# prj-beatrice/beatrice-vst

Hardware: AMD Instinct MI355X
Metric: audio frames/sec (24 kHz out, 10 ms hop) (higher is better)
Workload: dtype f32

## Files before the change

### beatrice-vst_amd/csrc/batch_tick.hip.h

```cpp
#pragma once

#ifdef BEATRICE_HIP_MEASUREMENT_BUILD
static unsigned long long g_tick_only_types = ~0ull;
#endif
template <int H>
bool tick_build_table_h(BeatriceBatch* b, const bool sparse) {
  using namespace tick;
  using O = Ops<H>;
  using Tab = typename O::Tab;
  using OpF2 = typename O::OpF2; using OpF3 = typename O::OpF3; using OpF4 = typename O::OpF4; using OpF5 = typename O::OpF5; using OpRB = typename O::OpRB;
  using OpOUT = typename O::OpOUT; using OpP1 = typename O::OpP1; using OpP23 = typename O::OpP23; using OpPOUT = typename O::OpPOUT; using OpINP = typename O::OpINP;
  using OpUP1 = typename O::OpUP1; using OpRES1A = typename O::OpRES1A; using OpRES1B = typename O::OpRES1B; using OpUP2 = typename O::OpUP2;
  using OpF4s = typename O::OpF4s; using OpF5s = typename O::OpF5s; using OpRBs = typename O::OpRBs; using OpP1s = typename O::OpP1s; using OpUP1s = typename O::OpUP1s;
  using T1 = typename O::T1; using T2 = typename O::T2; using T3 = typename O::T3; using T1s = typename O::T1s; using T2s = typename O::T2s;
  using GruQ = typename O::GruQ; using GruP = typename O::GruP; using GruQ1 = typename O::GruQ1; using GruP1 = typename O::GruP1;
  using GruQm = typename O::GruQm; using GruPm = typename O::GruPm;
  State& k = b->tk;
  if (sparse && !sparse_table_at(H)) { k.table_sparse_total = 0; return true; }
  auto tb = std::make_unique<typename O::Builder>();
  const PhoneWeights& pw = b->phone_m->w;
  const PitchWeights& qw = b->pitch_m->w;
  const WaveWeights& ww = b->wave_m->w;
  const PhoneState& ps = b->phone;
  const PitchState& qs = b->pitch;
  const WaveState& ws = b->wave;
  const int B = b->B;
  const Plan pl = k.plan;
#ifdef BEATRICE_HIP_MEASUREMENT_BUILD
  static const int drop = bhip::meas_env("BEATRICE_HIP_TICK_DROP") ? std::atoi(bhip::meas_env("BEATRICE_HIP_TICK_DROP")) : 0;
#else
  constexpr int drop = 0;
#endif
  auto keep = [](int group) { return ((drop >> group) & 1) == 0; };
#ifdef BEATRICE_HIP_MEASUREMENT_BUILD
  tb->only = g_tick_only_types;
#endif
  auto hp = [&](int) -> const int* { return nullptr; };
  auto conv = [&](const Ring& in, const Ring& out, const float* w, const float* bias, int stage) { return conv_args(in, out, w, bias, hp(stage), B); };
  static const int gru_passes_env = bhip::meas_env("BEATRICE_HIP_GRU_PASSES") ? std::atoi(bhip::meas_env("BEATRICE_HIP_GRU_PASSES")) : 0;
  const int gru_passes = gru_passes_env > 0 ? gru_passes_env : (B >= 512 ? 2 : 1);
  auto link_p = [&](int t) { return k.d_link_p + (size_t)t * B * 256; };
  auto link_q = [&](int t) { return k.d_link_q + (size_t)t * B * 128; };
  auto add_pgru = [&](int t) {
    if constexpr (H > 1) {
      GruArgs g{ps.rb[3], ps.h, pw.gru_wih, pw.gru_whh, pw.gru_bih, pw.gru_bhh, hp(Plan::PGRU), B, t, t + 1 < H ? link_p(t) : nullptr, t > 0 ? link_p(t - 1) : nullptr, k.h_link_dead, gru_passes};
      if (t == 0) tb->template add<T_PGRU>(GruP::info("phone.gru", g), g, GruP::grid(g), Plan::PGRU, keep(1), 19);
      else if (t == H - 1) tb->template add<T_PGRU1>(GruP1::info("phone.gru", g), g, GruP1::grid(g), Plan::PGRU, keep(1), 19);
      else if constexpr (H > 2) tb->template add<T_PGRUM>(GruPm::info("phone.gru", g), g, GruPm::grid(g), Plan::PGRU, keep(1), 19);
    }
  };
  auto add_qgru = [&](int t) {
    if constexpr (H > 1) {
      GruArgs g{qs.p[2], qs.h, qw.gru_wih, qw.gru_whh, qw.gru_bih, qw.gru_bhh, hp(Plan::QGRU), B, t, t + 1 < H ? link_q(t) : nullptr, t > 0 ? link_q(t - 1) : nullptr, k.h_link_dead, gru_passes};
      if (t == 0) tb->template add<T_QGRU>(GruQ::info("pitch.gru", g), g, GruQ::grid(g), Plan::QGRU, keep(1), 12);
      else if (t == H - 1) tb->template add<T_QGRU1>(GruQ1::info("pitch.gru", g), g, GruQ1::grid(g), Plan::QGRU, keep(1), 12);
      else if constexpr (H > 2) tb->template add<T_QGRUM>(GruQm::info("pitch.gru", g), g, GruQm::grid(g), Plan::QGRU, keep(1), 12);
    }
  };
  auto gru_at = [&](int point) {
    if constexpr (H == 2) { if (point == 2) add_pgru(1); if (point == 3) add_qgru(1); }
    if constexpr (H == 4) {
      if (point == 0) { add_pgru(1); add_qgru(1); }
      if (point == 1) { add_pgru(2); add_qgru(2); }
      if (point == 2) add_pgru(3);
      if (point == 3) add_qgru(3);
    }
  };
  add_pgru(0); add_qgru(0);
  if (!sparse) {
    { const ConvArgs a = conv(ps.f[3], ps.f[4], pw.f_w[3], pw.f_b[3], Plan::F5); tb->template add<T_F5>(OpF5::info("phone.f5", a), a, OpF5::grid(a), Plan::F5, keep(6), 30); }
    { const ConvArgs a = conv(qs.spec, qs.p[0], qw.p_w[0], qw.p_b[0], Plan::P1); tb->template add<T_P1>(OpP1::info("pitch.p1", a), a, OpP1::grid(a), Plan::P1, keep(2), 41); }
    { const ConvArgs a = conv(ps.f[2], ps.f[3], pw.f_w[2], pw.f_b[2], Plan::F4); tb->template add<T_F4>(OpF4::info("phone.f4", a), a, OpF4::grid(a), Plan::F4, keep(6), 28); }
    for (int i = 0; i < 4; ++i) {
      const ConvArgs a = conv(i == 0 ? ps.f[4] : ps.rb[i - 1], ps.rb[i], pw.rb_w[i], pw.rb_b[i], Plan::RB0 + i);
      tb->template add<T_RB>(OpRB::info("phone.rb", a), a, OpRB::grid(a), Plan::RB0 + i, keep(6), 39);
    }
  } else {
    { const ConvArgs a = conv(ps.f[3], ps.f[4], pw.f_w[3], pw.f_b[3], Plan::F5); tb->template add<T_F5S>(OpF5s::info("phone.f5", a), a, OpF5s::grid(a), Plan::F5, keep(6), 30); }
    { const ConvArgs a = conv(qs.spec, qs.p[0], qw.p_w[0], qw.p_b[0], Plan::P1); tb->template add<T_P1S>(OpP1s::info("pitch.p1", a), a, OpP1s::grid(a), Plan::P1, keep(2), 41); }
    { const ConvArgs a = conv(ps.f[2], ps.f[3], pw.f_w[2], pw.f_b[2], Plan::F4); tb->template add<T_F4S>(OpF4s::info("phone.f4", a), a, OpF4s::grid(a), Plan::F4, keep(6), 28); }
    for (int i = 0; i < 4; ++i) {
      const ConvArgs a = conv(i == 0 ? ps.f[4] : ps.rb[i - 1], ps.rb[i], pw.rb_w[i], pw.rb_b[i], Plan::RB0 + i);
      tb->template add<T_RBS>(OpRBs::info("phone.rb", a), a, OpRBs::grid(a), Plan::RB0 + i, keep(6), 39);
    }
  }
  for (int blk = 0; blk < B_NBLOCKS; ++blk) {
    const WaveState::Scratch& sc = ws.scr[blk];
    const int s0 = pl.blk(blk);
    const rc::BlockBArgs ba{sc.xa, ws.x[blk + 1], ww.q_w[blk], ww.q_b[blk], ww.o_w[blk], ww.o_b[blk], ws.d_kt[blk], ws.d_v[blk],
                            b->dev_view<int>(b->off.perm[blk]), b->dev_view<int>(b->off.tile_slot[blk]), hp(s0 + 1)};
    tb->template add<T_BLKB>(LaunchInfo{"wave.blk.b", 2.0 * B * H * (256.0 * 256 * 2 + 256.0 * 384 * 2), 4.0 * (2.0 * 256 * 256 + 2.0 * 256 * 384 + B * H * 3.0 * 256)}, ba,
                    dim3(ws.n_tiles_max, 1), s0 + 1, keep(5), 43.0);
    if (quads_on(b)) {
      const rc::BlockBqArgs bq{sc.xa, ws.x[blk + 1], ww.q_w[blk], ww.q_b[blk], ww.o_w[blk], ww.o_b[blk], ws.d_ktp[blk], ws.d_vp[blk],
                               b->dev_view<int>(b->off.qperm[blk]), b->dev_view<int>(b->off.qslot[blk]), hp(s0 + 1)};
      tb->template add<T_BLKBQ>(LaunchInfo{"wave.blk.bq", 0.0, 0.0}, bq, dim3(std::min(2 * ws.n_tiles_max, ws.n_slots), 1), s0 + 1, keep(5), 42.0);
    }
  }
  for (int blk = 0; blk < B_NBLOCKS; ++blk) {
    const rc::BlockAArgs aa{ws.x[blk], ws.scr[blk].xa, ww.c1_w[blk], ww.c1_b[blk], ww.c2_w[blk], ww.c2_b[blk], hp(pl.blk(blk)), B};
    switch (blk) {
      case 0: tb->template add<T_BLKA1>(rc::BlockAOp<1, H>::info(aa), aa, rc::BlockAOp<1, H>::grid(aa), pl.blk(blk), keep(5), 38); break;
      case 1: tb->template add<T_BLKA2>(rc::BlockAOp<2, H>::info(aa), aa, rc::BlockAOp<2, H>::grid(aa), pl.blk(blk), keep(5), 38); break;
      case 2: tb->template add<T_BLKA4>(rc::BlockAOp<4, H>::info(aa), aa, rc::BlockAOp<4, H>::grid(aa), pl.blk(blk), keep(5), 38); break;
      default: tb->template add<T_BLKA8>(rc::BlockAOp<8, H>::info(aa), aa, rc::BlockAOp<8, H>::grid(aa), pl.blk(blk), keep(5), 38); break;
    }
  }
  gru_at(0);
  { const VqArgs a{H, ps.raw, phone_vector_ring(ps), hp(Plan::VQ), ps.d_cbT, ps.d_cnorm, ps.d_vqk}; tb->template add<T_VQ>(LaunchInfo{"phone.vq", 0, 4.0 * B * H * 256}, a, dim3(B, 1), Plan::VQ, !ps.skip_vq, 9.0 * H, true); }
  {
    tst::StageArgs t1{}, t2{}, t3{};
    t1.in = ws.ya2; t1.out = ws.ya3; t2.in = ws.ya3; t2.out = ws.ya4; t3.in = ws.ya4;
    for (tst::StageArgs* t : {&t1, &t2, &t3}) { t->state = ws.tail.base; t->hop = nullptr; t->B = B; }
    t1.w[0] = ww.ra_w[1]; t1.b[0] = ww.ra_b[1]; t1.w[1] = ww.rb_w[1]; t1.b[1] = ww.rb_b[1]; t1.w[2] = ww.up_w[2]; t1.b[2] = ww.up_b[2];
    t2.w[0] = ww.ra_w[2]; t2.b[0] = ww.ra_b[2]; t2.w[1] = ww.rb_w[2]; t2.b[1] = ww.rb_b[2]; t2.w[2] = ww.up_w[3]; t2.b[2] = ww.up_b[3];
    t3.w[0] = ww.ra_w[3]; t3.b[0] = ww.ra_b[3]; t3.w[1] = ww.rb_w[3]; t3.b[1] = ww.rb_b[3];
    t3.fin_w = ww.fin_w; t3.fin_b = ww.fin_b; t3.d_out = ws.d_out; t3.io_stride = ws.io_stride;
    if (!sparse) {
      tb->template add<T_TAIL1>(T1::info(t1), t1, T1::grid(t1), pl.tail(), keep(4), 28, true);
      tb->template add<T_TAIL2>(T2::info(t2), t2, T2::grid(t2), pl.tail() + 1, keep(4), 11.5 * H, true);
    } else {
      tb->template add<T_TAIL1S>(T1s::info(t1), t1, T1s::grid(t1), pl.tail(), keep(4), 28, true);
      tb->template add<T_TAIL2S>(T2s::info(t2), t2, T2s::grid(t2), pl.tail() + 1, keep(4), 11.5 * H, true);
    }
    tb->template add<T_TAIL3>(T3::info(t3), t3, T3::grid(t3), pl.tail() + 2, keep(4), 6.5 * H, true);
  }
  gru_at(1);
  { PitchHeadArgs a = head_args(qw, qs); a.hop = hp(Plan::HEAD); tb->template add<T_HEAD>(head_info(qs), a, dim3((B + 7) / 8, 1), Plan::HEAD, keep(0), 7.5 * H); }
  { const ConvArgs a = conv(ps.f[1], ps.f[2], pw.f_w[1], pw.f_b[1], Plan::F3); tb->template add<T_F3>(OpF3::info("phone.f3", a), a, OpF3::grid(a), Plan::F3, keep(6), 15); }
  if (!sparse) { const ConvArgs a = conv(ws.x[4], ws.ya1, ww.up_w[0], ww.up_b[0], pl.up1()); tb->template add<T_UP1>(OpUP1::info("wave.up1", a), a, OpUP1::grid(a), pl.up1(), keep(7), 14); }
  else { const ConvArgs a = conv(ws.x[4], ws.ya1, ww.up_w[0], ww.up_b[0], pl.up1()); tb->template add<T_UP1S>(OpUP1s::info("wave.up1", a), a, OpUP1s::grid(a), pl.up1(), keep(7), 14); }
  { const ConvArgs a = conv(ws.yb1, ws.yc1, ww.rb_w[0], ww.rb_b[0], pl.up1() + 2); tb->template add<T_RES1B>(OpRES1B::info("wave.res1b", a), a, OpRES1B::grid(a), pl.up1() + 2, keep(7), 13); }
  { const ConvArgs a = conv(ws.ya1, ws.yb1, ww.ra_w[0], ww.ra_b[0], pl.up1() + 1); tb->template add<T_RES1A>(OpRES1A::info("wave.res1a", a), a, OpRES1A::grid(a), pl.up1() + 1, keep(7), 13); }
  { const ConvArgs a = conv(ws.yc1, ws.ya2, ww.up_w[1], ww.up_b[1], pl.up1() + 3); tb->template add<T_UP2>(OpUP2::info("wave.up2", a), a, OpUP2::grid(a), pl.up1() + 3, keep(7), 13); }
  { const ConvArgs a = conv(ps.f[0], ps.f[1], pw.f_w[0], pw.f_b[0], Plan::F2); tb->template add<T_F2>(OpF2::info("phone.f2", a), a, OpF2::grid(a), Plan::F2, keep(6), 15); }
  if constexpr (H == 1) { const GruArgs g{ps.rb[3], ps.h, pw.gru_wih, pw.gru_whh, pw.gru_bih, pw.gru_bhh, hp(Plan::PGRU), B, 0, nullptr, nullptr, nullptr, gru_passes}; tb->template add<T_PGRU>(GruP::info("phone.gru", g), g, GruP::grid(g), Plan::PGRU, keep(1), 19); }
  gru_at(2);
  { const ConvArgs a = conv(qs.h, qs.logits, qw.out_w, qw.out_b, Plan::POUT); tb->template add<T_POUT>(OpPOUT::info("pitch.out", a), a, OpPOUT::grid(a), Plan::POUT, keep(2), 11); }
  for (int i = 0; i < 2; ++i) {
    const ConvArgs a = conv(qs.p[i], qs.p[i + 1], qw.p_w[i + 1], qw.p_b[i + 1], Plan::P2 + i);
    tb->template add<T_P23>(OpP23::info("pitch.p23", a), a, OpP23::grid(a), Plan::P2 + i, keep(2), 10);
  }
  { const Ring phone_in{ws.d_phone, B_PHONE_CH, H, ws.front_slots}; ConvArgs a = conv(phone_in, ws.x[0], ww.inp_w, ww.inp_b, Plan::INP); a.res = ws.e; tb->template add<T_INP>(OpINP::info("wave.inp", a), a, OpINP::grid(a), Plan::INP, keep(3), 7.5); }
  if constexpr (H == 1) { const GruArgs g{qs.p[2], qs.h, qw.gru_wih, qw.gru_whh, qw.gru_bih, qw.gru_bhh, hp(Plan::QGRU), B, 0, nullptr, nullptr, nullptr, gru_passes}; tb->template add<T_QGRU>(GruQ::info("pitch.gru", g), g, GruQ::grid(g), Plan::QGRU, keep(1), 12); }
  gru_at(3);
  { FftArgs a = fft_args(qw, qs); a.hop = hp(Plan::FFT); tb->template add<T_FFT>(fft_info(qs), FftArgs2{a, B}, dim3((B + 1) / 2, H), Plan::FFT, keep(0), 8.7); }
  { const ConvArgs a = conv(ps.h, phone_out_ring(ps), pw.out_w, pw.out_b, Plan::OUT); tb->template add<T_OUT>(OpOUT::info("phone.out", a), a, OpOUT::grid(a), Plan::OUT, keep(3), 4.5); }
  { F1Args a = f1_args(pw, ps); a.hop = hp(Plan::F1); a.hop_publish = nullptr; a.hop_publish_wave = nullptr; tb->template add<T_F1>(f1_info(ps), F1Args2{a, B}, dim3((B + 1) / 2, H), Plan::F1, keep(0), 3.7); }
  { CondArgs a = cond_args(ww, ws); a.hop = hp(Plan::COND); a.hop_next_out = nullptr; tb->template add<T_COND>(cond_info(ws), a, dim3((B * H + 1) / 2, 1), Plan::COND, keep(0), 1.5); }
  if (!tb->ok) return false;
  static const int halves_mode = bhip::meas_env("BEATRICE_HIP_TICK_HALVES") ? std::atoi(bhip::meas_env("BEATRICE_HIP_TICK_HALVES")) : 2;
  {
    std::vector<fuse::WgDesc> desc;
    bool pinned[fuse::kMaxSpans];
    int group[fuse::kMaxSpans];
    for (int i = 0; i < tb->t.n_spans; ++i) {
      group[i] = -1;
      switch (tb->t.span[i].type) {
        case T_PGRU: case T_PGRU1: case T_PGRUM: pinned[i] = true; group[i] = 0; break;
        case T_QGRU: case T_QGRU1: case T_QGRUM: pinned[i] = true; group[i] = 1; break;
        case T_F2: case T_F3: case T_F4: case T_F5: case T_P1: case T_RB: case T_F4S: case T_F5S: case T_P1S: case T_RBS:
        case T_BLKA1: case T_BLKA2: case T_BLKA4: case T_BLKA8: case T_BLKB: case T_BLKBQ:
        case T_UP1: case T_UP1S: case T_RES1A: case T_RES1B: case T_UP2: case T_POUT: case T_P23: case T_INP: case T_OUT: pinned[i] = true; break;
        default: pinned[i] = false; break;
      }
    }
    if (halves_mode != 0 && !sparse) {
      desc = tb->two_halves(pinned, group, halves_mode == 4 ? 4 : 2);
    } else {
      desc = tb->in_span_order();
    }
    auto upload = [&](const std::vector<fuse::WgDesc>& v, DevBuf<fuse::WgDesc>& d_desc) {
      if (v.size() > d_desc.size() && !d_desc.alloc(v.size(), "tick dispatch order", false)) return false;
      if (!v.empty()) BHIP_TRY(hipMemcpy(d_desc, v.data(), sizeof(fuse::WgDesc) * v.size(), hipMemcpyHostToDevice));
      return true;
    };
    if (!sparse) {
      const std::vector<fuse::WgDesc> plain = tb->in_span_order();
      if (!upload(plain, k.d_desc_plain)) return false;
      k.table_total_plain = (int)plain.size();
      for (auto& row : k.range_n) for (int& n : row) n = 0;
      const int n_stages = pl.count();
      static const int range_halves_from = bhip::meas_env("BEATRICE_HIP_TICK_RANGE_HALVES") ? std::atoi(bhip::meas_env("BEATRICE_HIP_TICK_RANGE_HALVES")) : kRangeHalvesFrom;
      if (plain.size() <= 16384 && n_stages <= kMaxStages) {
        std::vector<fuse::WgDesc> all;
        for (int shape = 0; shape < 2; ++shape)
          for (int s0 = 0; s0 < n_stages; ++s0) {
            k.range_off[shape][s0] = all.size();
            const int occupied = shape == 0 ? s0 + 1 : n_stages - s0;
            if (halves_mode != 0 && occupied >= range_halves_from) {
              const std::vector<fuse::WgDesc> part = shape == 0 ? tb->two_halves(pinned, group, 2, 0, s0) : tb->two_halves(pinned, group, 2, s0, 255);
              all.insert(all.end(), part.begin(), part.end());
            } else {
              for (const fuse::WgDesc& d : plain) {
                const int stage = (d.arg >> 16) & 0xff;
                if (shape == 0 ? stage <= s0 : stage >= s0) all.push_back(d);
              }
            }
            k.range_n[shape][s0] = (int)(all.size() - k.range_off[shape][s0]);
          }
        if (!upload(all, k.d_desc_ranges)) return false;
      }
    }
    tb->t.total = (int)desc.size();
    if (!upload(desc, sparse ? k.d_desc_sparse : k.d_desc)) return false;
  }
  if (bhip::meas_env("BEATRICE_HIP_TICK_TRACE")) {
    if (!k.d_trace.alloc((size_t)3 * tb->t.total, "tick trace", false)) return false;
    tb->t.trace = k.d_trace;
// ... 530 lines not shown
```

### beatrice-vst_amd/csrc/rowchain.hip.h

```cpp
#pragma once
#include "meas_env.h"
#include <hip/hip_runtime.h>

#include <cstdlib>

#include "conv_gemm.hip.h"
#include "kernels_misc.hip.h"
#include "ring.h"
#include "spec_math.hip.h"

#ifdef RC_TIMING
__device__ unsigned long long* g_rc_stamps;
#define RC_STAMP(i) do { if (threadIdx.x == 0) g_rc_stamps[(size_t)blockIdx.x * 16 + (i)] = __builtin_readcyclecounter(); } while (0)
#else
#define RC_STAMP(i) do { } while (0)
#endif

namespace rc {

constexpr int NTHR = 512, NWAVE = 8;
constexpr int AS = B_HID + 8;
constexpr int TILE = 16 * AS;
constexpr int SS = B_KV_LEN + 8;
constexpr int STILE = 16 * SS;
__host__ __device__ constexpr int kpos(int k) { return (k & ~15) | ((k & 3) << 2) | ((k >> 2) & 3); }
constexpr int KSTEP = 4;
template <int ROWGROUPS >
__device__ __forceinline__ void piece_of(const int W, const int ln, int* r, int* q) {
  *r = 4 * (W % ROWGROUPS) + (ln >> 4); *q = 16 * (W / ROWGROUPS) + (ln & 15);
}
__device__ __forceinline__ int lane_koff(const int lane) { return 4 * (lane >> 4); }
__device__ __forceinline__ float4 lds_kblock(const float* __restrict__ p, const int kb) { return *reinterpret_cast<const float4*>(p + kb * 16); }
__device__ __forceinline__ void store_perm4(float* __restrict__ row, const int n0, const float v0, const float v1, const float v2, const float v3) {
  float* d = row + kpos(n0);
  d[0] = v0; d[4] = v1; d[8] = v2; d[12] = v3;
}

__device__ __forceinline__ void pin_pipeline() {
  asm volatile("" ::: "memory");
  __builtin_amdgcn_sched_barrier(0);
}
#ifndef RC_WSTREAM_GLOBAL
#define RC_WSTREAM_GLOBAL 1
#endif
struct WLane {
  const float4* p;
  __device__ static __forceinline__ WLane make(const float4* u, const int lane) { return WLane{u + lane}; }
  __device__ __forceinline__ WLane at(const size_t f4) const { return WLane{p + f4}; }
  __device__ __forceinline__ float4 kblock(const int kb) const { return p[(size_t)kb * 64]; }
};
using ::WGlobal;
#if RC_WSTREAM_GLOBAL
using WStream = WGlobal;
#else
using WStream = WLane;
#endif
struct NoGather { __device__ __forceinline__ void operator()() const {} };
template <int RT, int CG> __host__ __device__ constexpr int seg_depth() {
  constexpr int PREFETCH = 8;
  return RT == 1 ? (CG <= 2 ? PREFETCH : (CG <= 3 ? 4 : 2)) : (RT * CG <= 2 ? 8 : 4);
}
template <int RT, int CG, int KB, int D = seg_depth<RT, CG>(), class W, class Gather = NoGather>
__device__ __forceinline__ void mma_segment_rt(f32x4 (&acc)[RT][CG], const float* __restrict__ a, const int a_tile_stride,
                                               const W (&wf)[CG], Gather gather = Gather()) {
  static_assert(KB % D == 0, "segment length");
  float4 bq[D][CG];
  pin_pipeline();
#pragma unroll
  for (int d = 0; d < D; ++d)
#pragma unroll
    for (int c = 0; c < CG; ++c) bq[d][c] = wf[c].kblock(d);
  gather();
  float4 an[RT];
#pragma unroll
  for (int t = 0; t < RT; ++t) an[t] = lds_kblock(a + t * a_tile_stride, 0);
#pragma unroll
  for (int kb = 0; kb < KB; kb += D) {
#pragma unroll
    for (int d = 0; d < D; ++d) {
      float4 cur[CG];
#pragma unroll
      for (int c = 0; c < CG; ++c) cur[c] = bq[d][c];
      float4 av[RT];
#pragma unroll
      for (int t = 0; t < RT; ++t) av[t] = an[t];
      if (kb + d + D < KB) {
#pragma unroll
        for (int c = 0; c < CG; ++c) bq[d][c] = wf[c].kblock(kb + d + D);
      }
      if (kb + d + 1 < KB) {
#pragma unroll
        for (int t = 0; t < RT; ++t) an[t] = lds_kblock(a + t * a_tile_stride, kb + d + 1);
      }
      pin_pipeline();
#pragma unroll
      for (int t = 0; t < RT; ++t)
#pragma unroll
        for (int c = 0; c < CG; ++c) acc[t][c] = __builtin_amdgcn_mfma_f32_16x16x4f32(cur[c].x, av[t].x, acc[t][c], 0, 0, 0);
#pragma unroll
      for (int t = 0; t < RT; ++t)
#pragma unroll
        for (int c = 0; c < CG; ++c) acc[t][c] = __builtin_amdgcn_mfma_f32_16x16x4f32(cur[c].y, av[t].y, acc[t][c], 0, 0, 0);
#pragma unroll
      for (int t = 0; t < RT; ++t)
#pragma unroll
        for (int c = 0; c < CG; ++c) acc[t][c] = __builtin_amdgcn_mfma_f32_16x16x4f32(cur[c].z, av[t].z, acc[t][c], 0, 0, 0);
#pragma unroll
      for (int t = 0; t < RT; ++t)
#pragma unroll
        for (int c = 0; c < CG; ++c) acc[t][c] = __builtin_amdgcn_mfma_f32_16x16x4f32(cur[c].w, av[t].w, acc[t][c], 0, 0, 0);
    }
  }
}
template <int CG, int KB, class W>
__device__ __forceinline__ void mma_segment(f32x4 (&acc)[CG], const float* __restrict__ a, const W& wf, const size_t tile_stride) {
  W wfc[CG];
#pragma unroll
  for (int c = 0; c < CG; ++c) wfc[c] = wf.at(c * tile_stride);
  mma_segment_rt<1, CG, KB>(reinterpret_cast<f32x4 (&)[1][CG]>(acc), a, 0, wfc);
}

template <int NSEG, int CG, class Epi4>
__device__ __forceinline__ void layer256(const float* const (&seg)[NSEG], const int as, const float* __restrict__ w_packed,
                                         const int wave, const int lane, Epi4 epi4) {
  constexpr int K = NSEG * 256;
  const WStream wf = WStream::make(reinterpret_cast<const float4*>(w_packed) + (size_t)wave * (K / 16) * 64, lane);
  const size_t tile_stride = (size_t)NWAVE * (K / 16) * 64;
  f32x4 tot[CG];
#pragma unroll
  for (int s = 0; s < NSEG; ++s) {
    f32x4 acc[CG];
#pragma unroll
    for (int c = 0; c < CG; ++c) acc[c] = f32x4{0.f, 0.f, 0.f, 0.f};
    mma_segment<CG, 16>(acc, seg[s] + (lane & 15) * as + lane_koff(lane), wf.at((size_t)s * 16 * 64), tile_stride);
#pragma unroll
    for (int c = 0; c < CG; ++c) {
      if (s == 0) tot[c] = acc[c];
      else { tot[c][0] = tot[c][0] + acc[c][0]; tot[c][1] = tot[c][1] + acc[c][1]; tot[c][2] = tot[c][2] + acc[c][2]; tot[c][3] = tot[c][3] + acc[c][3]; }
    }
  }
#pragma unroll
  for (int c = 0; c < CG; ++c) epi4(lane & 15, (wave + NWAVE * c) * 16 + (lane >> 4) * 4, tot[c]);
}

template <int HOPS = 1>
__device__ __forceinline__ void load_tile(float* __restrict__ dst, const Ring& ring, const int* sid , const int pos, const int rel,
                                          const int tid, const int* rowhop = nullptr) {
  const float* gbase = as_global(ring.base);
#pragma unroll
  for (int i = 0; i < 2; ++i) {
    const int idx = tid + i * NTHR;
    int r, q;
    piece_of<4>(idx >> 6, idx & 63, &r, &q);
    const int b = sid[r];
    float4 v = make_float4(0.f, 0.f, 0.f, 0.f);
    if (b >= 0) v = *reinterpret_cast<const float4*>(gbase + (ring_index(ring, b / HOPS, rowhop != nullptr ? ring_pos(ring, rowhop[r]) : pos, rel + b % HOPS) + 4u * (unsigned)q));
    store_perm4(dst + r * AS, 4 * q, v.x, v.y, v.z, v.w);
  }
}
// ... 359 lines not shown
  static constexpr int LDS_FLOATS = kBlockBqLds;
  static constexpr double wg_cost() { return 30.0; }
  __device__ static __forceinline__ void run(const Args& a, int bx, int, float* lds) { block_bq_body<false, HOPS>(a, bx, lds); }
  template <bool RAG> __device__ static __forceinline__ void run_t(const Args& a, int bx, int, float* lds) { block_bq_body<RAG, HOPS>(a, bx, lds); }
};
using BlockBqOp = BlockBqOpH<1>;
constexpr int kConvRowsLds = 2 * TILE + 32;
template <int RT> constexpr int conv_rows_lds() { return 2 * RT * TILE + 48 * RT; }
template <class L, int COLS = 0, int RT = 1, bool RAG = false>
__device__ __forceinline__ void conv_rows_body(const ConvArgs& a, const int bx, const int by, float* __restrict__ lds) {
  constexpr int NCOL = COLS > 0 ? COLS : L::NOUT;
  static_assert(L::NOUT % NCOL == 0 && NCOL % 16 == 0, "column slabs");
  constexpr int K = L::K, P = L::P, NTL = NCOL / 16, CG = (NTL + NWAVE - 1) / NWAVE;
  constexpr int ROWS = 16 * RT;
  const int nt_base = by * NTL;
  constexpr int LAST = K - 256 * (P - 1);
  static_assert(K % 16 == 0 && LAST % 64 == 0 && L::NOUT % 16 == 0 && !L::GROUPED, "layer shape");
  float* slot[2] = {lds, lds + RT * TILE};
  int* rb_ = reinterpret_cast<int*>(lds + 2 * RT * TILE);
  const int tid = threadIdx.x, lane = tid & 63, wave = tid >> 6;
  const int hop = stepc::step(a.hop);
  if (hop < 0) return;
  WStream wfc[CG];
#pragma unroll
  for (int c = 0; c < CG; ++c) {
    const int nt = wave + NWAVE * c < NTL ? wave + NWAVE * c : NTL - 1;
    wfc[c] = WStream::make(reinterpret_cast<const float4*>(a.w) + (size_t)(nt_base + nt) * (K / 16) * 64, lane);
  }
  const int M = a.B * L::T;
  const bool rag = stepc::rag_t<RAG>();
  if (tid < ROWS) {
    const int m = bx * ROWS + tid;
    const int b = m < M ? m / L::T : -1;
    const int hr = b >= 0 ? stepc::of_t<RAG>(hop, b) : -1;
    rb_[tid] = hr >= 0 ? b : -1;
    rb_[ROWS + tid] = m < M ? m % L::T : 0;
    rb_[2 * ROWS + tid] = hr >= 0 ? hr : 0;
  }
  __syncthreads();
  const int pos_in = ring_pos(a.in, hop);
  int pr[2 * RT], pq[2 * RT], pb[2 * RT], pt[2 * RT];
#pragma unroll
  for (int i = 0; i < 2 * RT; ++i) {
    piece_of<4 * RT>(wave + NWAVE * i, lane, &pr[i], &pq[i]);
    pb[i] = rb_[pr[i]]; pt[i] = rb_[ROWS + pr[i]];
  }
  float4 nx[2 * RT];
  const float* in_base = as_global(a.in.base);
  auto load_seg = [&](int s) {
#pragma unroll
    for (int i = 0; i < 2 * RT; ++i) {
      const int kk = s * 256 + 4 * pq[i];
      const bool live = kk < K;
      const int j = live ? kk / L::CIN : 0, c = live ? kk % L::CIN : 0;
      nx[i] = make_float4(0.f, 0.f, 0.f, 0.f);
      if (live && pb[i] >= 0)
        nx[i] = *reinterpret_cast<const float4*>(in_base + (ring_index(a.in, pb[i], rag ? ring_pos(a.in, rb_[2 * ROWS + pr[i]]) : pos_in,
                                                                       (pt[i] + 1) * L::STRIDE - 1 - (L::KSZ - 1 - j) * L::DIL + a.rel_shift) + (unsigned)c));
    }
  };
  auto store_seg = [&](float* dst) {
#pragma unroll
    for (int i = 0; i < 2 * RT; ++i) {
      float4 v = nx[i];
      if constexpr (L::PRE == PRE_LRELU) { v.x = bsp::lrelu(v.x); v.y = bsp::lrelu(v.y); v.z = bsp::lrelu(v.z); v.w = bsp::lrelu(v.w); }
      store_perm4(dst + pr[i] * AS, 4 * pq[i], v.x, v.y, v.z, v.w);
    }
  };
  load_seg(0);
  store_seg(slot[0]);
  __syncthreads();
  f32x4 tot[RT][CG];
#pragma unroll
  for (int s = 0; s < P; ++s) {
    auto gather = [&] { if (s + 1 < P) load_seg(s + 1); };
    f32x4 acc[RT][CG];
#pragma unroll
    for (int t = 0; t < RT; ++t)
#pragma unroll
      for (int c = 0; c < CG; ++c) acc[t][c] = f32x4{0.f, 0.f, 0.f, 0.f};
    WStream wfs[CG];
#pragma unroll
    for (int c = 0; c < CG; ++c) wfs[c] = wfc[c].at((size_t)s * 16 * 64);
    const float* ap = slot[s & 1] + (lane & 15) * AS + lane_koff(lane);
    if (s + 1 < P) mma_segment_rt<RT, CG, 16>(acc, ap, TILE, wfs, gather);
    else mma_segment_rt<RT, CG, LAST / 16>(acc, ap, TILE, wfs, gather);
#pragma unroll
    for (int t = 0; t < RT; ++t)
#pragma unroll
      for (int c = 0; c < CG; ++c) {
        if (s == 0) tot[t][c] = acc[t][c];
        else { tot[t][c][0] = tot[t][c][0] + acc[t][c][0]; tot[t][c][1] = tot[t][c][1] + acc[t][c][1]; tot[t][c][2] = tot[t][c][2] + acc[t][c][2]; tot[t][c][3] = tot[t][c][3] + acc[t][c][3]; }
      }
    if (s + 1 < P) {
      store_seg(slot[(s + 1) & 1]);
      __syncthreads();
    }
  }
  const int pos_out = ring_pos(a.out, hop), R_out = a.out.n * a.out.m;
  int pos_res = 0, R_res = 0;
  if constexpr (L::RES) { pos_res = ring_pos(a.res, hop); R_res = a.res.n * a.res.m; }
  float4 bias_n[CG];
#pragma unroll
  for (int c = 0; c < CG; ++c) {
    const int nt = wave + NWAVE * c < NTL ? wave + NWAVE * c : NTL - 1;
    bias_n[c] = L::EPI == EPI_BIAS ? *reinterpret_cast<const float4*>(a.bias + (nt_base + nt) * 16 + (lane >> 4) * 4) : make_float4(0.f, 0.f, 0.f, 0.f);
  }
#pragma unroll
  for (int t = 0; t < RT; ++t) {
    const int r = 16 * t + (lane & 15);
    const int rb = rb_[r], rf = rb_[ROWS + r];
    int po = pos_out, pr = pos_res;
    if (rag) {
      const int hr = rb_[2 * ROWS + r];
      po = ring_pos(a.out, hr);
      if constexpr (L::RES) pr = ring_pos(a.res, hr);
    }
    float rs = 1.0f;
    if constexpr (L::EPI == EPI_ROWSCALE) rs = a.rowscale[(rb < 0 ? 0 : rb) * L::T + rf];
#pragma unroll
    for (int c = 0; c < CG; ++c) {
      if (wave + NWAVE * c >= NTL) continue;
      const int n0 = (nt_base + wave + NWAVE * c) * 16 + (lane >> 4) * 4;
      float v[4];
#pragma unroll
      for (int e = 0; e < 4; ++e) v[e] = tot[t][c][e];
      if constexpr (L::EPI == EPI_BIAS) { v[0] = v[0] + bias_n[c].x; v[1] = v[1] + bias_n[c].y; v[2] = v[2] + bias_n[c].z; v[3] = v[3] + bias_n[c].w; }
      if constexpr (L::EPI == EPI_SCALE) { for (int e = 0; e < 4; ++e) v[e] = v[e] * a.scale; }
      if constexpr (L::EPI == EPI_ROWSCALE) { for (int e = 0; e < 4; ++e) v[e] = v[e] * rs; }
      if constexpr (L::ACT == ACT_GELU) {
        const bsp::f32x2 g0 = bsp::gelu2(bsp::f32x2{v[0], v[1]}), g1 = bsp::gelu2(bsp::f32x2{v[2], v[3]});
        v[0] = g0.x; v[1] = g0.y; v[2] = g1.x; v[3] = g1.y;
      }
      if (rb < 0) continue;
      if constexpr (L::RES) {
        const float4 x = *reinterpret_cast<const float4*>(a.res.base + ((unsigned)(rb * R_res + pr) * (unsigned)a.res.C + (unsigned)(rf * L::NOUT + n0)));
        v[0] = x.x + v[0]; v[1] = x.y + v[1]; v[2] = x.z + v[2]; v[3] = x.w + v[3];
      }
      *reinterpret_cast<float4*>(a.out.base + ((unsigned)(rb * R_out + po) * (unsigned)a.out.C + (unsigned)(rf * L::NOUT + n0))) = make_float4(v[0], v[1], v[2], v[3]);
    }
  }
}
template <class L, int COLS = 0, int RT = 1>
struct ConvRowsOp {
  using Args = ConvArgs;
  static constexpr int NTHR = rc::NTHR;
  static constexpr int LDS_FLOATS = conv_rows_lds<RT>();
  static inline dim3 grid(const ConvArgs& a) { return dim3((a.B * L::T + 16 * RT - 1) / (16 * RT), COLS > 0 ? L::NOUT / COLS : 1); }
  static inline bhip::LaunchInfo info(const char* name, const ConvArgs& a) { return ConvOp<L, TileCfg<1, 1, 1, 2, 1>>::info(name, a); }
  __device__ static __forceinline__ void run(const ConvArgs& a, int bx, int by, float* lds) { conv_rows_body<L, COLS, RT>(a, bx, by, lds); }
  template <bool RAG> __device__ static __forceinline__ void run_t(const ConvArgs& a, int bx, int by, float* lds) { conv_rows_body<L, COLS, RT, RAG>(a, bx, by, lds); }
};

struct NopOp {
  struct Args { int unused; };
  static constexpr int NTHR = 64;
  static constexpr int LDS_FLOATS = 0;
  __device__ static __forceinline__ void run(const Args&, int, int, float*) {}
  template <bool RAG> __device__ static __forceinline__ void run_t(const Args&, int, int, float*) {}
};

template <class L, int COLS, int RT>
static __global__ __launch_bounds__(NTHR, 4) void conv_rows_kernel(const ConvArgs a) {
  __shared__ __attribute__((aligned(16))) float lds[conv_rows_lds<RT>()];
  conv_rows_body<L, COLS, RT>(a, blockIdx.x, blockIdx.y, lds);
}
template <class L, int COLS = 0, int RT = 2>
static inline void launch_conv_rows(const char* name, const ConvArgs& a, hipStream_t stream) {
  using Op = ConvRowsOp<L, COLS, RT>;
  bhip::launch_site(Op::info(name, a), stream, [&] { hipLaunchKernelGGL((conv_rows_kernel<L, COLS, RT>), Op::grid(a), dim3(NTHR), 0, stream, a); });
}

}

template <class L>
static inline void launch_many_rows(const char* name, const ConvArgs& a, hipStream_t s) {
  constexpr int LAST = L::K - 256 * (L::P - 1);
  constexpr bool ok = !L::GROUPED && L::K % 16 == 0 && LAST % 64 == 0 && L::NOUT % 16 == 0;
  if constexpr (ok) {
    static const bool off = bhip::meas_env("BEATRICE_HIP_NO_CONVROWS") != nullptr;
    if (!off) {
      constexpr int COLS = (L::NOUT % 128 == 0 && (L::NOUT > 256 || (L::NOUT == 256 && L::K >= 768))) ? 128 : 0;
      rc::launch_conv_rows<L, COLS, 2>(name, a, s);
      return;
    }
  }
  launch_conv<L, TL>(name, a, 0, s);
}
```

### beatrice-vst_amd/csrc/tick.hip.h

```cpp
#pragma once
#include <type_traits>

#include "chain_layers.hip.h"
#include "fuse.hip.h"
#include "hip_owned.h"
#include "rowchain.hip.h"
#include "tail_stages.hip.h"
#include "tick_reset.hip.h"

namespace tick {

constexpr int kRangeHalvesFrom = 99;
constexpr int kMaxStages = 32, kRing = 64, kMaxCopies = 16;

struct Copy { unsigned char* dst; const unsigned char* src; int bytes; };
constexpr int kCopyChunk = 4096;
struct Prolog {
  int n_stages;
  int hop[kMaxStages], io[kMaxStages];
  int n_copies;
  Copy copy[kMaxCopies];
  int first_chunk[kMaxCopies + 1];
};
static __global__ __launch_bounds__(256) void prologue_kernel(const Prolog p) {
  int c = 0;
  while (c + 1 < p.n_copies && (int)blockIdx.x >= p.first_chunk[c + 1]) ++c;
  const Copy cp = p.copy[c];
  const int at = ((int)blockIdx.x - p.first_chunk[c]) * kCopyChunk + (int)threadIdx.x * 16;
  if (at + 16 <= cp.bytes) *reinterpret_cast<uint4*>(cp.dst + at) = *reinterpret_cast<const uint4*>(cp.src + at);
}

using namespace bhip;
using namespace wave_layers;
constexpr int kRbCols = 128;
constexpr int kGruRt = 2, kMidRt = 2, kRbRt = 2, kP1Rt = kMidRt;
constexpr int kF3Rt = 1;

constexpr bool sparse_table_at(int H) { return H == 1; }

enum BodyType {
  T_F1, T_FFT, T_F2, T_F3, T_F4, T_F5, T_P1, T_RB, T_P23, T_POUT, T_HEAD, T_OUT, T_COND, T_INP, T_UP1, T_RES1A, T_RES1B, T_UP2,
  T_QGRU, T_PGRU, T_VQ, T_TAIL1, T_TAIL2, T_TAIL3, T_BLKA1, T_BLKA2, T_BLKA4, T_BLKA8, T_BLKB, T_BLKBQ,
  T_F4S, T_F5S, T_RBS, T_P1S, T_UP1S, T_TAIL1S, T_TAIL2S, T_QGRU1, T_PGRU1, T_QGRUM, T_PGRUM, T_COUNT
};
template <int H>
struct Ops {
  using PL = PhoneLayers<H>;
  using QL1 = PitchLayers<H>;
  using OpF2 = rc::ConvRowsOp<typename PL::F2, 0, kMidRt>;
  using OpF3 = rc::ConvRowsOp<typename PL::F3, 0, kF3Rt>;
  using OpF4 = rc::ConvRowsOp<typename PL::F4, kRbCols, kRbRt>;
  using OpF5 = rc::ConvRowsOp<typename PL::F5, kRbCols, kRbRt>;
  using OpRB = rc::ConvRowsOp<typename PL::RBL, kRbCols, kRbRt>;
  using OpOUT = rc::ConvRowsOp<typename PL::OUTL>;
  using OpP1 = rc::ConvRowsOp<typename QL1::P1, 0, kP1Rt>;
  using OpP23 = rc::ConvRowsOp<typename QL1::P23>;
  using OpPOUT = rc::ConvRowsOp<typename QL1::POUT>;
  using OpINP = rc::ConvRowsOp<INP<H>>;
  using OpUP1 = rc::ConvRowsOp<UP<256, 128, 5, H>, 128, kMidRt>;
  using OpRES1A = rc::ConvRowsOp<RES<128, 1, 5 * H>, 0, kMidRt>;
  using OpRES1B = rc::ConvRowsOp<RES<128, 3, 5 * H>, 0, kMidRt>;
  using OpUP2 = rc::ConvRowsOp<UP<128, 64, 4, 5 * H>, 0, kMidRt>;
  template <class Op> using Sparse = std::conditional_t<sparse_table_at(H), Op, fuse::Absent<Op>>;
  using OpF4s = Sparse<rc::ConvRowsOp<typename PL::F4, kRbCols, 1>>;
  using OpF5s = Sparse<rc::ConvRowsOp<typename PL::F5, kRbCols, 1>>;
  using OpRBs = Sparse<rc::ConvRowsOp<typename PL::RBL, kRbCols, 1>>;
  using OpP1s = Sparse<rc::ConvRowsOp<typename QL1::P1, 0, 1>>;
  using OpUP1s = Sparse<rc::ConvRowsOp<UP<256, 128, 5, H>, 128, 1>>;
  static constexpr int NSUB = H > 2 ? H / 2 : 1;
  using T1 = tst::T1OpS<(H == 1 ? tst::kT1Streams : (H == 2 ? 2 : 1)), H>;
  using T2 = tst::T2OpS<(H == 1 ? tst::kT2Streams : 1), H, NSUB>;
  using T3 = tst::T3OpS<(H == 1 ? tst::kT3Streams : 1), H, NSUB>;
  using T1s = Sparse<tst::T1OpS<(H == 1 ? 2 : 1), H>>;
  using T2s = Sparse<tst::T2OpS<(H == 1 ? 2 : 1), H, NSUB>>;
  static_assert(H <= 4, "link arrays: tick::State");
  using GruQ = GruOp<128, 128, kGruRt, (H > 1 ? 1 : 0)>;
  using GruP = GruOp<256, 256, kGruRt, (H > 1 ? 1 : 0)>;
  using GruQ1 = std::conditional_t<H == 1, rc::NopOp, GruOp<128, 128, kGruRt, 2>>;
  using GruP1 = std::conditional_t<H == 1, rc::NopOp, GruOp<256, 256, kGruRt, 2>>;
  using GruQm = std::conditional_t<H <= 2, rc::NopOp, GruOp<128, 128, kGruRt, 3>>;
  using GruPm = std::conditional_t<H <= 2, rc::NopOp, GruOp<256, 256, kGruRt, 3>>;
  using Vq = std::conditional_t<H == 1, VqOp, VqRowsOp<H>>;
  template <class... Ms> struct List { using Tab = fuse::Table<Ms...>; using Builder = fuse::TableBuilder<Ms...>; };
  using L = List<
      fuse::Many<F1Op2, 1>, fuse::Many<FftOp2, 1>, fuse::Many<OpF2, 1>, fuse::Many<OpF3, 1>, fuse::Many<OpF4, 1>, fuse::Many<OpF5, 1>,
      fuse::Many<OpP1, 1>, fuse::Many<OpRB, 4>, fuse::Many<OpP23, 2>, fuse::Many<OpPOUT, 1>, fuse::Many<HeadOp8, 1>,
      fuse::Many<OpOUT, 1>, fuse::Many<CondOp2, 1>, fuse::Many<OpINP, 1>, fuse::Many<OpUP1, 1>, fuse::Many<OpRES1A, 1>,
      fuse::Many<OpRES1B, 1>, fuse::Many<OpUP2, 1>, fuse::Many<GruQ, 1>, fuse::Many<GruP, 1>,
      fuse::Many<Vq, 1>, fuse::Many<T1, 1>, fuse::Many<T2, 1>, fuse::Many<T3, 1>, fuse::Many<rc::BlockAOp<1, H>, 1>, fuse::Many<rc::BlockAOp<2, H>, 1>,
      fuse::Many<rc::BlockAOp<4, H>, 1>, fuse::Many<rc::BlockAOp<8, H>, 1>, fuse::Many<rc::BlockBOpH<H>, 4>, fuse::Many<rc::BlockBqOpH<H>, 4>,
      fuse::Many<OpF4s, 1>, fuse::Many<OpF5s, 1>, fuse::Many<OpRBs, 4>, fuse::Many<OpP1s, 1>, fuse::Many<OpUP1s, 1>, fuse::Many<T1s, 1>, fuse::Many<T2s, 1>,
      fuse::Many<GruQ1, 1>, fuse::Many<GruP1, 1>, fuse::Many<GruQm, 2>, fuse::Many<GruPm, 2>>;
  using Tab = typename L::Tab;
  using Builder = typename L::Builder;
};

struct Plan {
  static constexpr int F1 = 0, F2 = 1, F3 = 2, F4 = 3, FFT = 3, F5 = 4, P1 = 4, RB0 = 5, P2 = 5, QGRU = 7, POUT = 8, PGRU = 9, HEAD = 9,
                       OUT = 10, COND = 10, VQ = 11, INP = 12, BLK0 = 13;
  static constexpr int per_block = 2;
  int blk(int b) const { return BLK0 + per_block * b; }
  int up1() const { return blk(B_NBLOCKS); }
  int tail() const { return up1() + 4; }
  int count() const { return tail() + 3; }
};
constexpr int kMaxHops = 4;
static_assert(Plan::BLK0 + Plan::per_block * B_NBLOCKS + 7 <= kMaxStages && kMaxStages + 2 <= kRing && kMaxStages <= fuse::kMaxStepPairs, "stage bookkeeping");

struct Consumer {
  int stage;
  size_t off, bytes;
  unsigned char* dst;
  int held;
};

struct State {
  bool on = false;
  DevBuf<unsigned char> d_table;
  int table_total = 0;
  DevBuf<unsigned char> d_table_sparse;
  int table_sparse_total = 0;
  double table_flops = 0, table_bytes = 0;
  DevBuf<fuse::WgDesc> d_desc;
  DevBuf<fuse::WgDesc> d_desc_sparse;
  DevBuf<fuse::WgDesc> d_desc_plain;
  int table_total_plain = 0;
  DevBuf<fuse::WgDesc> d_desc_ranges;
  size_t range_off[2][kMaxStages] = {};
  int range_n[2][kMaxStages] = {};
  DevBuf<unsigned long long> d_trace;
  bool table_dirty = true;
  DevBuf<unsigned char> d_snap;
  static constexpr int kStaging = 16;
  StagedRing<unsigned char> stage;
  size_t snap_bytes = 0;
  long long tick = 0, n_fed = 0, last_feed_tick = -1000;
  long long fed_step[kRing];
  int snap_of_step[kRing], hop_of_step[kRing], io_of_step[kRing];
  int snap_cur = -1, snap_next = 0;
  std::vector<Consumer> consumers;
  Plan plan;
  bool ragged = false;
  int row = 0;
  std::vector<int> hop_s;
  DevBuf<int> d_hopv;
  StagedRing<int> hopv;
  bool step_ragged[kRing] = {};
  DevBuf<FreezeRing> d_ring_table;
  int n_ring_table = 0;
  DevBuf<int> d_shift;
  DevBuf<unsigned long long> d_link_q;
  DevBuf<unsigned long long> d_link_p;
  PinnedBuf<int> h_link_dead;
  struct Travelling { int stream, counter; long long tick; };
  std::vector<unsigned char> reset_pending;
  bool any_reset_pending = false;
  std::vector<Travelling> resets;
  DevBuf<ResetRing> d_reset_rings;
  int n_reset_rings = 0;
  std::vector<int> reset_stage;
  std::vector<unsigned char> reset_spare;
  std::vector<int> reset_m;
  static constexpr int kResetStaging = 8;
  StagedRing<int> reset_list;
  size_t reset_list_ints = 0;
  long long reset_serial = 0, reset_launches = 0;
  DevBuf<float> d_gru_keep;
};

}
```

Baseline: 4.827 million.

## Add row-tiled MFMA GRU cell op for multi-hop chained GRU stages

Introduces a GruRowsOp that stages x and h rows into LDS and computes all three gates with MFMA segments over 16*RT batch rows per workgroup. It also fuses the gate nonlinearities and the cross-hop link publish/acquire into the same op. The multi-hop GRU variants (H>1) switch from the older GruOp to this op, and their scheduling cost estimates in the fused table are retuned. The aim is better weight reuse and a cheaper per-hop GRU step. The new code adds LDS pressure and changes the grid shape, which may shift the balance of the persistent schedule.

Result: faster. 5.008 million, median of 6 (+3.8%).

```diff
diff --git a/beatrice-vst_amd/csrc/batch_tick.hip.h b/beatrice-vst_amd/csrc/batch_tick.hip.h
--- a/beatrice-vst_amd/csrc/batch_tick.hip.h
+++ b/beatrice-vst_amd/csrc/batch_tick.hip.h
@@ -37,6 +37,7 @@
 #endif
   auto hp = [&](int) -> const int* { return nullptr; };
   auto conv = [&](const Ring& in, const Ring& out, const float* w, const float* bias, int stage) { return conv_args(in, out, w, bias, hp(stage), B); };
+  constexpr double kGruRowsCostP = 25, kGruRowsCostQ = H == 2 ? 14 : 17;
   static const int gru_passes_env = bhip::meas_env("BEATRICE_HIP_GRU_PASSES") ? std::atoi(bhip::meas_env("BEATRICE_HIP_GRU_PASSES")) : 0;
   const int gru_passes = gru_passes_env > 0 ? gru_passes_env : (B >= 512 ? 2 : 1);
   auto link_p = [&](int t) { return k.d_link_p + (size_t)t * B * 256; };
@@ -44,17 +45,17 @@
   auto add_pgru = [&](int t) {
     if constexpr (H > 1) {
       GruArgs g{ps.rb[3], ps.h, pw.gru_wih, pw.gru_whh, pw.gru_bih, pw.gru_bhh, hp(Plan::PGRU), B, t, t + 1 < H ? link_p(t) : nullptr, t > 0 ? link_p(t - 1) : nullptr, k.h_link_dead, gru_passes};
-      if (t == 0) tb->template add<T_PGRU>(GruP::info("phone.gru", g), g, GruP::grid(g), Plan::PGRU, keep(1), 19);
-      else if (t == H - 1) tb->template add<T_PGRU1>(GruP1::info("phone.gru", g), g, GruP1::grid(g), Plan::PGRU, keep(1), 19);
-      else if constexpr (H > 2) tb->template add<T_PGRUM>(GruPm::info("phone.gru", g), g, GruPm::grid(g), Plan::PGRU, keep(1), 19);
+      if (t == 0) tb->template add<T_PGRU>(GruP::info("phone.gru", g), g, GruP::grid(g), Plan::PGRU, keep(1), H == 2 ? kGruRowsCostP : 19);
+      else if (t == H - 1) tb->template add<T_PGRU1>(GruP1::info("phone.gru", g), g, GruP1::grid(g), Plan::PGRU, keep(1), kGruRowsCostP);
+      else if constexpr (H > 2) tb->template add<T_PGRUM>(GruPm::info("phone.gru", g), g, GruPm::grid(g), Plan::PGRU, keep(1), kGruRowsCostP);
     }
   };
   auto add_qgru = [&](int t) {
     if constexpr (H > 1) {
       GruArgs g{qs.p[2], qs.h, qw.gru_wih, qw.gru_whh, qw.gru_bih, qw.gru_bhh, hp(Plan::QGRU), B, t, t + 1 < H ? link_q(t) : nullptr, t > 0 ? link_q(t - 1) : nullptr, k.h_link_dead, gru_passes};
-      if (t == 0) tb->template add<T_QGRU>(GruQ::info("pitch.gru", g), g, GruQ::grid(g), Plan::QGRU, keep(1), 12);
-      else if (t == H - 1) tb->template add<T_QGRU1>(GruQ1::info("pitch.gru", g), g, GruQ1::grid(g), Plan::QGRU, keep(1), 12);
-      else if constexpr (H > 2) tb->template add<T_QGRUM>(GruQm::info("pitch.gru", g), g, GruQm::grid(g), Plan::QGRU, keep(1), 12);
+      if (t == 0) tb->template add<T_QGRU>(GruQ::info("pitch.gru", g), g, GruQ::grid(g), Plan::QGRU, keep(1), kGruRowsCostQ);
+      else if (t == H - 1) tb->template add<T_QGRU1>(GruQ1::info("pitch.gru", g), g, GruQ1::grid(g), Plan::QGRU, keep(1), kGruRowsCostQ);
+      else if constexpr (H > 2) tb->template add<T_QGRUM>(GruQm::info("pitch.gru", g), g, GruQm::grid(g), Plan::QGRU, keep(1), kGruRowsCostQ);
     }
   };
   auto gru_at = [&](int point) {
diff --git a/beatrice-vst_amd/csrc/rowchain.hip.h b/beatrice-vst_amd/csrc/rowchain.hip.h
--- a/beatrice-vst_amd/csrc/rowchain.hip.h
+++ b/beatrice-vst_amd/csrc/rowchain.hip.h
@@ -5,6 +5,7 @@
 #include <cstdlib>
 
 #include "conv_gemm.hip.h"
+#include "fused_small.hip.h"
 #include "kernels_misc.hip.h"
 #include "ring.h"
 #include "spec_math.hip.h"
@@ -670,6 +671,150 @@
   template <bool RAG> __device__ static __forceinline__ void run_t(const ConvArgs& a, int bx, int by, float* lds) { conv_rows_body<L, COLS, RT, RAG>(a, bx, by, lds); }
 };
 
+template <int IN, int H, int RT> constexpr int gru_rows_lds() { return 16 * RT * (IN + 8) + 16 * RT * (H + 8); }
+template <int IN, int H, bool RAG = false, int LINK = 0, int RT = 2>
+__device__ __forceinline__ void gru_rows_body(const GruArgs& a, const int bx, const int by, float* __restrict__ lds) {
+  constexpr int XS = IN + 8, HS = H + 8, ROWS = 16 * RT, CT = NWAVE / RT;
+  constexpr int NPX = ROWS * (IN / 4) / NTHR, NPH = ROWS * (H / 4) / NTHR;
+  static_assert(RT == 1 || RT == 2, "row tiles");
+  static_assert(NWAVE % (4 * RT) == 0, "piece_of: wave-loads w and w + NWAVE i hold the same rows (the gather takes a thread's row once)");
+  static_assert(IN % 64 == 0 && H % 64 == 0 && H % (16 * CT) == 0 && NPX >= 1 && NPH >= 1 && (XS / 4) % 16 == 2 && (HS / 4) % 16 == 2, "cell shape");
+  float* xs = lds;
+  float* hs = lds + ROWS * XS;
+  const int tid = threadIdx.x, lane = tid & 63, wave = __builtin_amdgcn_readfirstlane(tid >> 6);
+  const int hop = __builtin_amdgcn_readfirstlane(stepc::step(a.hop));
+  if (hop < 0) return;
+  const bool rag = stepc::rag_t<RAG>();
+  const int px = __builtin_amdgcn_readfirstlane(ring_pos(a.x, hop)), ph = __builtin_amdgcn_readfirstlane(ring_pos(a.h, hop));
+  asm volatile("" : : "s"(px), "s"(ph));
+  const int b0 = bx * ROWS;
+  const int tile = by * CT + wave % CT, rt = wave / CT;
+  WStream wx[3], wh[3];
+#pragma unroll
+  for (int g = 0; g < 3; ++g) {
+    wx[g] = WStream::make(reinterpret_cast<const float4*>(a.wih) + (size_t)(g * (H / 16) + tile) * (IN / 16) * 64, lane);
+    wh[g] = WStream::make(reinterpret_cast<const float4*>(a.whh) + (size_t)(g * (H / 16) + tile) * (H / 16) * 64, lane);
+  }
+  auto gather = [&] {
+    int r, q0;
+    piece_of<4 * RT>(wave, lane, &r, &q0);
+    const int b = b0 + r;
+    const int hr = b < a.B ? (rag ? stepc::hopv[b] : hop) : -1;
+    float4 vx[NPX], vh[NPH];
+    {
+      const float* xb = as_global(a.x.base);
+      const unsigned xi = ring_index(a.x, b, rag ? ring_pos(a.x, hr) : px, a.t);
+#pragma unroll
+      for (int i = 0; i < NPX; ++i) {
+        int ri, q;
+        piece_of<4 * RT>(wave + NWAVE * i, lane, &ri, &q);
+        vx[i] = make_float4(0.f, 0.f, 0.f, 0.f);
+        if (hr >= 0) vx[i] = *reinterpret_cast<const float4*>(xb + (xi + 4u * (unsigned)q));
+      }
+    }
+    if constexpr ((LINK & 2) != 0) {
+      const unsigned long long* gp = a.link_in + (size_t)b * H;
+      unsigned long long gv[NPH][4];
+#pragma unroll
+      for (int i = 0; i < NPH; ++i) {
+        int ri, q;
+        piece_of<4 * RT>(wave + NWAVE * i, lane, &ri, &q);
+#pragma unroll
+        for (int j = 0; j < 4; ++j) gv[i][j] = hr >= 0 ? __hip_atomic_load(gp + 4 * q + j, __ATOMIC_RELAXED, __HIP_MEMORY_SCOPE_AGENT) : 0ull;
+      }
+#pragma unroll
+      for (int i = 0; i < NPX; ++i) {
+        int ri, q;
+        piece_of<4 * RT>(wave + NWAVE * i, lane, &ri, &q);
+        store_perm4(xs + r * XS, 4 * q, vx[i].x, vx[i].y, vx[i].z, vx[i].w);
+      }
+#pragma unroll
+      for (int i = 0; i < NPH; ++i) {
+        int ri, q;
+        piece_of<4 * RT>(wave + NWAVE * i, lane, &ri, &q);
+        float f[4];
+#pragma unroll
+        for (int j = 0; j < 4; ++j)
+          f[j] = hr < 0 ? 0.0f : ((int)(gv[i][j] >> 32) == hop + 1 ? __uint_as_float((unsigned)gv[i][j]) : glink::acquire(gp + 4 * q + j, hop + 1, a.link_dead));
+        store_perm4(hs + r * HS, 4 * q, f[0], f[1], f[2], f[3]);
+      }
+    } else {
+      const float* hb = as_global(a.h.base);
+      const unsigned hi = ring_index(a.h, b, rag ? ring_pos(a.h, hr) : ph, a.t - 1);
+#pragma unroll
+      for (int i = 0; i < NPH; ++i) {
+        int ri, q;
+        piece_of<4 * RT>(wave + NWAVE * i, lane, &ri, &q);
+        vh[i] = make_float4(0.f, 0.f, 0.f, 0.f);
+        if (hr >= 0) vh[i] = *reinterpret_cast<const float4*>(hb + (hi + 4u * (unsigned)q));
+      }
+#pragma unroll
+      for (int i = 0; i < NPX; ++i) {
+        int ri, q;
+        piece_of<4 * RT>(wave + NWAVE * i, lane, &ri, &q);
+        store_perm4(xs + r * XS, 4 * q, vx[i].x, vx[i].y, vx[i].z, vx[i].w);
+      }
+#pragma unroll
+      for (int i = 0; i < NPH; ++i) {
+        int ri, q;
+        piece_of<4 * RT>(wave + NWAVE * i, lane, &ri, &q);
+        store_perm4(hs + r * HS, 4 * q, vh[i].x, vh[i].y, vh[i].z, vh[i].w);
+      }
+    }
+    __syncthreads();
+  };
+  f32x4 ax[1][3], ah[1][3];
+#pragma unroll
+  for (int g = 0; g < 3; ++g) { ax[0][g] = f32x4{0.f, 0.f, 0.f, 0.f}; ah[0][g] = f32x4{0.f, 0.f, 0.f, 0.f}; }
+  const int row = 16 * rt + (lane & 15);
+  mma_segment_rt<1, 3, IN / 16>(ax, xs + row * XS + lane_koff(lane), 0, wx, gather);
+  mma_segment_rt<1, 3, H / 16>(ah, hs + row * HS + lane_koff(lane), 0, wh);
+  const int b = b0 + row;
+  const int hr = b < a.B ? (rag ? stepc::hopv[b] : hop) : -1;
+  if (hr < 0) return;
+  const int n0 = 16 * tile + 4 * (lane >> 4);
+  float bi[3][4], bh[3][4];
+#pragma unroll
+  for (int g = 0; g < 3; ++g) {
+    const float4 vi = *reinterpret_cast<const float4*>(a.bih + g * H + n0), vh = *reinterpret_cast<const float4*>(a.bhh + g * H + n0);
+    bi[g][0] = vi.x; bi[g][1] = vi.y; bi[g][2] = vi.z; bi[g][3] = vi.w;
+    bh[g][0] = vh.x; bh[g][1] = vh.y; bh[g][2] = vh.z; bh[g][3] = vh.w;
+  }
+  const float* hprev = hs + row * HS + kpos(n0);
+  float zz[4], pre[4], nn[4], hv[4];
+#pragma unroll
+  for (int e = 0; e < 4; ++e) {
+    const float gi_r = ax[0][0][e] + bi[0][e], gi_z = ax[0][1][e] + bi[1][e], gi_n = ax[0][2][e] + bi[2][e];
+    const float gh_r = ah[0][0][e] + bh[0][e], gh_z = ah[0][1][e] + bh[1][e], gh_n = ah[0][2][e] + bh[2][e];
+    const bsp::f32x2 rz = bsp::sigmoid2(bsp::f32x2{gi_r + gh_r, gi_z + gh_z});
+    zz[e] = rz.y;
+    pre[e] = bsp::fma(rz.x, gh_n, gi_n);
+  }
+  {
+    const bsp::f32x2 t0 = bsp::tanh2(bsp::f32x2{pre[0], pre[1]}), t1 = bsp::tanh2(bsp::f32x2{pre[2], pre[3]});
+    nn[0] = t0.x; nn[1] = t0.y; nn[2] = t1.x; nn[3] = t1.y;
+  }
+#pragma unroll
+  for (int e = 0; e < 4; ++e) hv[e] = bsp::fma(zz[e], hprev[KSTEP * e] - nn[e], nn[e]);
+  *reinterpret_cast<float4*>(ring_frame(a.h, b, rag ? ring_pos(a.h, hr) : ph, a.t) + n0) = make_float4(hv[0], hv[1], hv[2], hv[3]);
+  if constexpr ((LINK & 1) != 0) {
+#pragma unroll
+    for (int e = 0; e < 4; ++e) glink::publish(a.link_out + (size_t)b * H + n0 + e, hv[e], hop + 1);
+  }
+}
+template <int IN, int H, int LINK = 0, int RT = 2>
+struct GruRowsOp {
+  using Args = GruArgs;
+  static constexpr int NTHR = rc::NTHR;
+  static constexpr int LDS_FLOATS = gru_rows_lds<IN, H, RT>();
+  static inline dim3 grid(const GruArgs& a) { return dim3((a.B + 16 * RT - 1) / (16 * RT), H / (16 * (NWAVE / RT))); }
+  static inline bhip::LaunchInfo info(const char* name, const GruArgs& a) {
+    return bhip::LaunchInfo{name, 2.0 * a.B * (IN + H) * 3.0 * H, 4.0 * ((IN + H) * 3.0 * H + a.B * (IN + 2.0 * H))};
+  }
+  __device__ static __forceinline__ void run(const GruArgs& a, int bx, int by, float* lds) { gru_rows_body<IN, H, false, LINK, RT>(a, bx, by, lds); }
+  template <bool RAG> __device__ static __forceinline__ void run_t(const GruArgs& a, int bx, int by, float* lds) { gru_rows_body<IN, H, RAG, LINK, RT>(a, bx, by, lds); }
+};
+
 struct NopOp {
   struct Args { int unused; };
   static constexpr int NTHR = 64;
diff --git a/beatrice-vst_amd/csrc/tick.hip.h b/beatrice-vst_amd/csrc/tick.hip.h
--- a/beatrice-vst_amd/csrc/tick.hip.h
+++ b/beatrice-vst_amd/csrc/tick.hip.h
@@ -33,7 +33,7 @@
 using namespace bhip;
 using namespace wave_layers;
 constexpr int kRbCols = 128;
-constexpr int kGruRt = 2, kMidRt = 2, kRbRt = 2, kP1Rt = kMidRt;
+constexpr int kMidRt = 2, kRbRt = 2, kP1Rt = kMidRt;
 constexpr int kF3Rt = 1;
 
 constexpr bool sparse_table_at(int H) { return H == 1; }
@@ -74,12 +74,12 @@
   using T1s = Sparse<tst::T1OpS<(H == 1 ? 2 : 1), H>>;
   using T2s = Sparse<tst::T2OpS<(H == 1 ? 2 : 1), H, NSUB>>;
   static_assert(H <= 4, "link arrays: tick::State");
-  using GruQ = GruOp<128, 128, kGruRt, (H > 1 ? 1 : 0)>;
-  using GruP = GruOp<256, 256, kGruRt, (H > 1 ? 1 : 0)>;
-  using GruQ1 = std::conditional_t<H == 1, rc::NopOp, GruOp<128, 128, kGruRt, 2>>;
-  using GruP1 = std::conditional_t<H == 1, rc::NopOp, GruOp<256, 256, kGruRt, 2>>;
-  using GruQm = std::conditional_t<H <= 2, rc::NopOp, GruOp<128, 128, kGruRt, 3>>;
-  using GruPm = std::conditional_t<H <= 2, rc::NopOp, GruOp<256, 256, kGruRt, 3>>;
+  using GruQ = std::conditional_t<H == 1, GruOp<128, 128, 2, 0>, rc::GruRowsOp<128, 128, 1>>;
+  using GruP = std::conditional_t<H == 2, rc::GruRowsOp<256, 256, 1>, GruOp<256, 256, 2, (H > 1 ? 1 : 0)>>;
+  using GruQ1 = std::conditional_t<H == 1, rc::NopOp, rc::GruRowsOp<128, 128, 2>>;
+  using GruP1 = std::conditional_t<H == 1, rc::NopOp, rc::GruRowsOp<256, 256, 2>>;
+  using GruQm = std::conditional_t<H <= 2, rc::NopOp, rc::GruRowsOp<128, 128, 3>>;
+  using GruPm = std::conditional_t<H <= 2, rc::NopOp, rc::GruRowsOp<256, 256, 3>>;
   using Vq = std::conditional_t<H == 1, VqOp, VqRowsOp<H>>;
   template <class... Ms> struct List { using Tab = fuse::Table<Ms...>; using Builder = fuse::TableBuilder<Ms...>; };
   using L = List<
```
